# dell-research-harvard/effocr

Measured on AMD Instinct MI355X. Metric: glyph-crops/sec end-to-end (encode+kNN), 224x224 bs=1024, higher is better.
Workload: dtype bf16; 1 GPU; BASELINE configs[1]: vit_small_patch16_224 encoder (bf16 MFMA operands, fp32 accumulate/residual/LN/softmax), 1024x3x224x224 fp32 crops per GPU resident in HBM, 10000-row fp32 IndexFlatIP, k=10; seeded random-init weights; crops_per_gpu=1024, global_batch=1024, index_rows=10000, k=10, parallelism=1024 crops per GPU, weights+index replicated

## Files before the change

### effocr_amd/_lib.py

```python
import ctypes
import os
import subprocess
import threading

_HERE = os.path.dirname(os.path.abspath(__file__))
_CSRC = os.path.join(_HERE, "csrc")
SO_PATH = os.environ.get("EFFOCR_HIP_LIB") or os.path.join(_HERE, "libeffocr_hip.so")
SO_PATH_AB = os.path.join(_HERE, "libeffocr_hip_ab.so")

ABI_VERSION = 9
PREC = {"bf16": 0, "fp16": 1, "fp32": 2}
EPI = {"bias": 0, "bias_gelu": 1, "bias_resid": 2}

_lock = threading.Lock()
_lib = None
_loaded = {}


class EffOCRHipError(RuntimeError):
    pass


def build(force=False, verbose=False, ab=True):
    so = os.path.join(_HERE, "libeffocr_hip.so")
# ... 84 lines not shown
        "effocr_letterbox": (i32, [vp, i32, i32, i64, i32, i32, i32, i32, i32, i32, i32, f32p, vp]),
        "effocr_nms_workspace_bytes": (sz, [i32, i32]),
        "effocr_nms_batch_workspace_bytes": (sz, [i32, i32, i32]),
        "effocr_nms": (i32, [f32p, i32, i32, c.c_float, c.c_float, i32, i32, c.c_float, i32, f32p, vp, vp, sz, vp]),
        "effocr_nms_batch": (i32, [f32p, i32, i32, i32, c.c_float, c.c_float, i32, i32, c.c_float, i32, f32p, vp, vp, sz, vp]),
        "effocr_parse_char_boxes": (i32, [f32p, vp, i32, i32, i32, i32, i32, i32, f32p, vp, vp, vp, vp]),
        "effocr_op_linear": (i32, [i32, i32, vp, vp, f32p, f32p, vp, i32, i32, i32, vp]),
        "effocr_op_layernorm": (i32, [i32, f32p, i64, i32, f32p, f32p, c.c_float, vp, vp]),
        "effocr_op_attention": (i32, [i32, vp, vp, i32, i32, i32, vp]),
        "effocr_op_linear_blocked": (i32, [i32, i32, vp, vp, f32p, f32p, vp, i32, i32, i32, i32, vp]),
        "effocr_op_mlp_blocked": (i32, [i32, f32p, f32p, f32p, c.c_float, vp, f32p, vp, f32p, f32p, i32, i32, i32, i32, vp, sz, vp]),
        "effocr_op_mlp_ln_blocked": (i32, [i32, f32p, f32p, f32p, c.c_float, vp, f32p, vp, f32p, f32p, f32p, f32p, vp, i32, i32, i32, i32, vp, sz, vp]),
        "effocr_op_proj_mlp_blocked": (i32, [i32, f32p, vp, vp, f32p, f32p, f32p, c.c_float, vp, f32p, vp, f32p, f32p, i32, i32, i32, i32, vp, sz, vp]),
        "effocr_op_qkv_attn_blocked": (i32, [i32, vp, vp, f32p, vp, i32, i32, i32, i32, vp]),
        "effocr_op_layernorm_blocked": (i32, [i32, f32p, i64, i32, f32p, f32p, c.c_float, vp, vp]),
    }
    for name, (res, args) in sig.items():
        if os.environ.get("EFFOCR_HIP_LIB") and not hasattr(lib, name):
            def _absent(*a, _n=name, **k):
                raise EffOCRHipError(f"{_n} is not exported by the library EFFOCR_HIP_LIB points at")
            setattr(lib, name, _absent)
            continue
        fn = getattr(lib, name)
        fn.restype = res
        fn.argtypes = args
    return sig


EXPORTS = None

# ... 380 lines not shown
```

### effocr_amd/csrc/api.hip

```cpp
#include "../../include/effocr_hip.h"
#include "enc_core.hpp"


#include <math.h>
#include <algorithm>
#include <string.h>
#include <map>
#include <memory>
#include <string>
#include <vector>

namespace effocr {

namespace {

struct Param { std::string name; std::vector<int64_t> shape; int64_t numel; std::vector<float> data; bool set; };

struct VitCfg { int D, depth, heads, mlp; };
struct VitLayerOff { size_t ln1w, ln1b, qkvb, projb, ln2w, ln2b, fc1b, fc2b, qkvw, projw, fc1w, fc2w;
                     size_t qkvw_b, projw_b, fc1w_b, fc2w_b, projw_pp, fc2w_pp, projb_p, fc2b_p, qkvw_bv, qkvb_v;
                     size_t qkvw_bf, qkv_s, qkv_c, fc1w_bf, fc1_s, fc1_c; };
struct ConvSpec { std::string w, bn; int cin, cout, k, stride, pad; size_t w_off, b_off; };
struct CnxBlockOff { size_t dww, dwb, lnw, lnb, w1, b1, w2, b2, gamma; };
struct CnxStageOff { int C, Cp, depth; size_t dslnw, dslnb, dsw, dsb; std::vector<CnxBlockOff> blocks; };

}
}

using namespace effocr;

struct effocr_encoder {
  std::string arch;
  bool is_vit = false;
  int img = 224, prec = PREC_BF16, D = 0;
  std::vector<Param> params;
  std::map<std::string, int> index;
  VitCfg vit{};
  int T = 0, P = 0;
  size_t off_clspos0 = 0, off_pos = 0, off_patchb = 0, off_normw = 0, off_normb = 0, off_patchw = 0, off_patchw_b = 0;
  std::vector<VitLayerOff> layers;
  std::vector<ConvSpec> convs;
  bool is_cnx = false;
  std::vector<CnxStageOff> cnx;
  size_t cnx_stemw = 0, cnx_stemb = 0, cnx_stemlnw = 0, cnx_stemlnb = 0, cnx_headw = 0, cnx_headb = 0;
  bool is_mnv = false;
  MnvNet mnv{};
  size_t wbytes = 0;
  const char* wdev = nullptr;
  int debug = 0;
  int cls_only_last = 1;
  int mlp_stagger_min_rounds = 2;
  int mlp_tail_first = 96;
  int mlp_stagger = 2500;
  int use_projf = 1;
  int use_qkvattn = 1;
  int qa_min_batch = 1;
  int qa_hsplit = 0;
  int use_patchf = 1;
  int use_mlp = 1;
  int use_gemm3 = 1;
  int use_lnfold = 1;
  int tail_split = 1;
  int split6 = 1;
  int pair_parts = 1;
  int mlp_pair = 0;
  int use_blocked = 1;
  int use_gemm2 = 1;
  int panel_rows = 128;
  int use_panel = 1;
  int chunk = 0;
  int call_size_invariant = 0;
  int prof_mode = 0;
// ... 60 lines not shown
    L.ln2w = a.take((size_t)D * 4); L.ln2b = a.take((size_t)D * 4);
    L.fc1b = a.take((size_t)mlp * 4); L.fc2b = a.take((size_t)D * 4);
  }
  e->off_normw = a.take((size_t)D * 4);
  e->off_normb = a.take((size_t)D * 4);
  e->off_patchw = a.take((size_t)D * 768 * es);
  for (int i = 0; i < depth; ++i) {
    VitLayerOff& L = e->layers[i];
    L.qkvw = a.take((size_t)3 * D * D * es);
    L.projw = a.take((size_t)D * D * es);
    L.fc1w = a.take((size_t)mlp * D * es);
    L.fc2w = a.take((size_t)D * mlp * es);
  }
  if (e->prec != PREC_FP32) {
    e->off_patchw_b = a.take((size_t)D * 768 * es);
    for (int i = 0; i < depth; ++i) {
      VitLayerOff& L = e->layers[i];
      L.fc2w_b = a.take((size_t)D * mlp * es);
      L.fc2w_pp = a.take((size_t)D * mlp * es);
      L.projw_pp = a.take((size_t)D * D * es);
      L.projb_p = a.take((size_t)D * 4);
      L.fc2b_p = a.take((size_t)D * 4);
      L.qkvw_bv = a.take((size_t)3 * D * D * es);
      L.qkvb_v = a.take((size_t)3 * D * 4);
      {
        L.qkvw_b = a.take((size_t)3 * D * D * es);
        L.projw_b = a.take((size_t)D * D * es);
        L.fc1w_b = a.take((size_t)mlp * D * es);
        L.qkvw_bf = a.take((size_t)3 * D * D * es); L.qkv_s = a.take((size_t)3 * D * 4); L.qkv_c = a.take((size_t)3 * D * 4);
        L.fc1w_bf = a.take((size_t)mlp * D * es); L.fc1_s = a.take((size_t)mlp * 4); L.fc1_c = a.take((size_t)mlp * 4);
// ... 391 lines not shown
  }
  const int cls = prof_class(e, name);
  const size_t slot = e->prof_used++;
  const bool clk = e->prof_mode == 1 && slot < effocr_encoder::PROF_CLK_SLOTS &&
                   (e->prof_clk || hipMalloc(&e->prof_clk, effocr_encoder::PROF_CLK_SLOTS * 8192 * sizeof(unsigned long long)) == hipSuccess && hipMemset(e->prof_clk, 0, effocr_encoder::PROF_CLK_SLOTS * 8192 * sizeof(unsigned long long)) == hipSuccess);
  if (clk) (void)clock_sample(e->prof_clk + slot * 8192, s);
  (void)hipEventRecord(e->prof_pool[slot].first, s);
  const int rc = launch();
  (void)hipEventRecord(e->prof_pool[slot].second, s);
  if (clk) (void)clock_sample(e->prof_clk + slot * 8192 + 4096, s);
  e->prof_rec.push_back({cls, (int)slot});
  e->prof_work[cls] += work;
  return rc;
}

struct VitWs { size_t status, x, xn, qkv, att, h, stats, total, rows, hbytes; };
VitWs vit_ws(const effocr_encoder* e, int B) {
  const size_t M = align_up((size_t)B * e->T, 128), D = e->vit.D, es = prec_esize(e->prec);
  Alloc a; VitWs w;
  w.rows = M;
  w.status = a.take(256);
  w.x = a.take(M * D * 4);
  w.xn = a.take(M * D * es);
  w.qkv = a.take(M * 3 * D * es);
  w.att = a.take(M * D * es);
  size_t hb = M * e->vit.mlp * es, pb = (size_t)B * e->P * 768 * es;
  w.hbytes = hb > pb ? hb : pb;
  {
    const size_t cus = (size_t)device_cus(), np = M / 128, tail = np % cus;
    const size_t split = (tail && tail * 6 <= cus) ? 6 : (tail && tail * 4 <= cus) ? 4 : (tail && tail * 2 <= cus) ? 2 : 0;
// ... 14 lines not shown
  void* xn = ws + w.xn; void* qkv = ws + w.qkv; void* att = ws + w.att; void* hb = ws + w.h;
  auto F = [&](size_t off) { return reinterpret_cast<const float*>(wb + off); };
  int rc;
  const double Md = (double)M, Dd = (double)D, Hd = (double)e->vit.mlp;
  const bool panel = e->use_panel && panel_gemm_supported(prec, 3 * D, D) && panel_gemm_supported(prec, e->vit.mlp, D);
  const bool g2 = e->use_gemm2 && gemm2_supported(prec, D, e->vit.mlp);
  const bool g2p = e->use_gemm2 && gemm2_supported(prec, D, 768);
  const bool g3all = !panel && e->use_gemm3 && gemm3_supported(prec, 3 * D, D) && gemm3_supported(prec, D, D) &&
                     gemm3_supported(prec, e->vit.mlp, D) && gemm3_supported(prec, D, e->vit.mlp);
  const int blk = (e->use_blocked && g2p && ((panel && g2) || g3all)) ? 1 : 0;
  const bool mlpf = blk && panel && e->use_mlp && mlp_fused_supported(prec, D, e->vit.mlp);
  const bool projf = mlpf && e->use_projf;
  const bool qaf = blk && panel && mlpf && qkv_attn_supported(prec, D, T) && (e->use_qkvattn == 2 || (e->use_qkvattn == 1 && (e->call_size_invariant || B >= e->qa_min_batch)));
  const bool g3 = blk && e->use_gemm3 && gemm3_supported(prec, D, e->vit.mlp);
  const bool patchf = blk && e->use_patchf && patch_embed_fused_supported(prec, D);
  if (!patchf && (rc = timed(e, "im2col_patch16", 0.0, s, [&] { return im2col_patch16(prec, x, x16, B, e->img, e->img, hb, s); }))) return rc;
  int* status = reinterpret_cast<int*>(ws + w.status);
  if (!patchf && (rc = set_cls_rows(F(e->off_clspos0), xs, B, T, D, blk, nullptr, s))) return rc;
  GemmArgs g{};
  if (patchf) {
    PatchArgs pa{};
    pa.x = x; pa.x16 = x16; pa.B = B; pa.H = e->img; pa.W = e->img; pa.Wb = wb + e->off_patchw_b; pa.bias = F(e->off_patchb); pa.pos = F(e->off_pos);
    pa.out = xs; pa.D = D; pa.P = Pn; pa.cls = F(e->off_clspos0);
    if ((rc = timed(e, "patch_embed_fused", 2.0 * B * Pn * Dd * 768.0, s, [&] { return patch_embed_fused(prec, pa, s); }))) return rc;
  } else {
  g.X = hb; g.ldx = 768; g.W = wb + e->off_patchw; g.ldw = 768; g.bias = F(e->off_patchb);
  g.out = xs; g.ldo = D; g.pos = F(e->off_pos); g.M = B * Pn; g.N = D; g.K = 768; g.P = Pn; g.blk_out = blk;
  if ((rc = timed(e, "gemm_patch_embed", 2.0 * B * Pn * Dd * 768.0, s, [&] { return g2p ? gemm2_nt(prec, EPI_PATCH, g, s) : gemm_nt(prec, EPI_PATCH, g, s); }))) return rc;
  }
  const float* cls_x = nullptr;
  bool xn_ready = false;
  for (int i = 0; i < e->vit.depth; ++i) {
    const VitLayerOff& L = e->layers[i];
    if (panel) {
      {
      PanelArgs p{};
      if (qaf) {
        if (!xn_ready && (rc = timed(e, "layernorm", 0.0, s, [&] { return layernorm_rows_blocked(prec, xs, M, D, F(L.ln1w), F(L.ln1b), 1e-6f, xn, s); }))) return rc;
        xn_ready = false;
        QkvAttnArgs q{};
        q.xn = xn; q.Wb = wb + L.qkvw_bv; q.bias = F(L.qkvb_v); q.out = att;
        q.B = B; q.T = T; q.D = D; q.rows_alloc = (int64_t)w.rows; q.hsplit = e->qa_hsplit;
        q.cls_only = (i + 1 == e->vit.depth && e->cls_only_last && projf) ? 1 : 0;
        const bool cls_k = q.cls_only && D == 384 && T > 192;
        const double qa_work = cls_k ? 2.0 * Md * 2.0 * Dd * Dd + 2.0 * (32.0 * B) * Dd * Dd + 4.0 * B * e->vit.heads * 32.0 * T * 64.0
                                     : 2.0 * Md * 3.0 * Dd * Dd + 4.0 * B * e->vit.heads * (double)T * T * 64.0;
// ... 402 lines not shown
}

size_t effocr_encoder_weights_bytes(const effocr_encoder_t* enc) { return enc ? enc->wbytes : 0; }

int effocr_encoder_upload(effocr_encoder_t* enc, void* weights_dev, size_t bytes) {
  if (!enc || !weights_dev) return fail(EFFOCR_EINVAL, "upload: NULL argument");
  if (bytes < enc->wbytes) return fail(EFFOCR_EWORKSPACE, "upload: weight buffer too small");
  for (const Param& p : enc->params)
    if (!p.set) return fail(EFFOCR_ESTATE, "upload: parameter '" + p.name + "' was never set");
  std::vector<char> blob(enc->wbytes, 0);
  if (enc->is_vit) pack_vit(enc, blob); else if (enc->is_cnx) pack_convnext(enc, blob); else if (enc->is_mnv) pack_mobilenetv3(enc, blob);
  else pack_resnet(enc, blob);
  const hipError_t er = hipMemcpy(weights_dev, blob.data(), enc->wbytes, hipMemcpyHostToDevice);
  if (er != hipSuccess) return fail(EFFOCR_EHIP, std::string("upload: hipMemcpy: ") + hipGetErrorString(er));
  enc->wdev = static_cast<const char*>(weights_dev);
  return EFFOCR_OK;
}

size_t effocr_encoder_workspace_bytes(const effocr_encoder_t* enc, int batch) {
  if (!enc || batch <= 0) return 0;
  if (enc->is_cnx) return convnext_ws(enc, cnx_chunk(enc, batch)).total;
  if (enc->is_mnv) return mnv3_ws(enc, mnv3_chunk(enc, batch)).total;
  if (!enc->is_vit) return resnet_ws(enc, batch).total;
  return vit_ws(enc, (enc->chunk > 0 && enc->chunk < batch) ? enc->chunk : batch).total;
}

int effocr_encoder_set_option(effocr_encoder_t* enc, const char* name, int value) {
  if (!enc || !name) return fail(EFFOCR_EINVAL, "set_option: NULL argument");
  const std::string n = name;
  if (n == "use_panel") { enc->use_panel = value; return EFFOCR_OK; }
  if (n == "debug") { enc->debug = value; return EFFOCR_OK; }
  if (n == "use_gemm2") { enc->use_gemm2 = value; return EFFOCR_OK; }
  if (n == "use_blocked") { enc->use_blocked = value; return EFFOCR_OK; }
  if (n == "tail_split") { enc->tail_split = value; return EFFOCR_OK; }
  if (n == "split6") { enc->split6 = value; return EFFOCR_OK; }
  if (n == "mlp_pair") { enc->mlp_pair = value; return EFFOCR_OK; }
  if (n == "pair_parts") { enc->pair_parts = value; return EFFOCR_OK; }
  if (n == "use_gemm3") { enc->use_gemm3 = value; return EFFOCR_OK; }
  if (n == "use_lnfold") { enc->use_lnfold = value; return EFFOCR_OK; }
  if (n == "use_mlp") { enc->use_mlp = value; return EFFOCR_OK; }
  if (n == "use_qkvattn") { enc->use_qkvattn = value; return EFFOCR_OK; }
  if (n == "qa_min_batch") { enc->qa_min_batch = value; return EFFOCR_OK; }
  if (n == "qa_hsplit") { enc->qa_hsplit = value; return EFFOCR_OK; }
  if (n == "use_patchf") { enc->use_patchf = value; return EFFOCR_OK; }
  if (n == "use_projf") { enc->use_projf = value; return EFFOCR_OK; }
  if (n == "cls_only_last") { enc->cls_only_last = value; return EFFOCR_OK; }
  if (n == "mlp_stagger_min_rounds") { enc->mlp_stagger_min_rounds = value < 1 ? 1 : value; return EFFOCR_OK; }
  if (n == "mlp_tail_first") { enc->mlp_tail_first = value < 0 ? 0 : value & ~7; return EFFOCR_OK; }
  if (n == "mlp_stagger") { enc->mlp_stagger = value < 0 ? 0 : value; return EFFOCR_OK; }
  if (n == "panel_rows") { if (value != 64 && value != 128) return fail(EFFOCR_EINVAL, "set_option: panel_rows must be 64 or 128"); enc->panel_rows = value; return EFFOCR_OK; }
  if (n == "call_size_invariant") {
    if (value != 0 && value != 1) return fail(EFFOCR_EINVAL, "set_option: call_size_invariant must be 0 or 1");
    enc->call_size_invariant = value; return EFFOCR_OK;
  }
  if (n == "chunk") { if (value < 0) return fail(EFFOCR_EINVAL, "set_option: chunk < 0"); enc->chunk = value; return EFFOCR_OK; }
  return fail(EFFOCR_EINVAL, "set_option: unknown option '" + n + "'");
}

int effocr_encoder_set_chunk(effocr_encoder_t* enc, int crops_per_chunk) {
// ... 331 lines not shown
  if (batch > 0 && (!xn_blk_dev || !wqkv_blk_dev || !bias_dev || !out_blk_dev))
    return fail(EFFOCR_EINVAL, "op_qkv_attn_blocked: NULL device pointer");
  if (batch < 0 || tokens < 1) return fail(EFFOCR_EINVAL, "op_qkv_attn_blocked: bad batch / tokens");
  QkvAttnArgs q{};
  q.xn = xn_blk_dev; q.Wb = wqkv_blk_dev; q.bias = bias_dev; q.out = out_blk_dev;
  q.B = batch; q.T = tokens; q.D = d; q.rows_alloc = rows_alloc;
  return qkv_attn_fused(precision, q, S(stream));
}

int effocr_op_layernorm_blocked(int out_precision, const float* x_blk_dev, int64_t rows, int d, const float* gamma_dev,
                                const float* beta_dev, float eps, void* out_blk_dev, void* stream) {
  if (rows > 0 && (!x_blk_dev || !gamma_dev || !beta_dev || !out_blk_dev)) return fail(EFFOCR_EINVAL, "op_layernorm_blocked: NULL device pointer");
  return layernorm_rows_blocked(out_precision, x_blk_dev, rows, d, gamma_dev, beta_dev, eps, out_blk_dev, S(stream));
}

int effocr_op_layernorm(int out_precision, const float* x_dev, int64_t rows, int d, const float* gamma_dev,
                        const float* beta_dev, float eps, void* out_dev, void* stream) {
  return layernorm_rows(out_precision, x_dev, rows, d, gamma_dev, beta_dev, eps, out_dev, S(stream));
}

int effocr_op_attention(int precision, const void* qkv_dev, void* out_dev, int batch, int tokens, int heads, void* stream) {
  return attention(precision, qkv_dev, out_dev, batch, tokens, heads, 0, S(stream));
}

}
```

### effocr_amd/csrc/kernels.hpp

```cpp
#pragma once
#include "common.hpp"

namespace effocr {

enum { PREC_BF16 = 0, PREC_FP16 = 1, PREC_FP32 = 2 };
enum { EPI_BIAS = 0, EPI_BIAS_GELU = 1, EPI_BIAS_RESID = 2, EPI_PATCH = 3,
       EPI_BIAS_SCALE_RESID = 4,
       EPI_BIAS_F32 = 5 };

static inline int prec_esize(int prec) { return prec == PREC_FP32 ? 4 : 2; }

struct GemmArgs {
  const void* X; int64_t ldx;
  const void* W; int64_t ldw;
  const float* bias;
  void* out; int64_t ldo;
  const float* resid; int64_t ldr;
  const float* pos;
  int M, N, K;
  int P;
  int blk_x;
  int blk_out;
  const void* Wblk;
  int rows_alloc;
// ... 43 lines not shown
  int cls_only;
  int img0;
  int hsplit;
};
bool qkv_attn_supported(int prec, int D, int T);
int qkv_attn_fused(int prec, const QkvAttnArgs& a, hipStream_t s);

struct PatchArgs {
  const void* x; int B, H, W;
  int x16;
  const void* Wb;
  const float* bias; const float* pos;
  const float* cls;
  float* out;
  int D, P;
};
bool patch_embed_fused_supported(int prec, int D);
int patch_embed_fused(int prec, const PatchArgs& a, hipStream_t s);

enum { PRO_COPY = 0, PRO_LN = 1 };
struct PanelArgs {
  const void* A; int64_t lda;
  const float* gamma; const float* beta; float eps;
  const void* W;
  const float* bias;
  void* out; int64_t ldo;
  const float* resid; int64_t ldr;
  int M, N, K;
  unsigned long long* dbg;
  int debug;
  int blk_a;
  int blk_out;
// ... 109 lines not shown
```

### effocr_amd/csrc/ln.hpp

```cpp
#pragma once
#include "common.hpp"

namespace effocr {

template <int G> __device__ __forceinline__ float group_sum(float v) {
#pragma unroll
  for (int o = G / 2; o >= 1; o >>= 1) v += __shfl_xor(v, o, 64);
  return v;
}

template <int G, int V>
__device__ __forceinline__ void ln_apply(const f32x4 (&v)[V], int sub, const float* __restrict__ gamma,
                                         const float* __restrict__ beta, float eps, f32x4 (&y)[V]) {
  constexpr int D = 4 * G * V;
  float s = 0.f;
#pragma unroll
  for (int i = 0; i < V; ++i) s += (v[i][0] + v[i][1]) + (v[i][2] + v[i][3]);
  const float mean = group_sum<G>(s) * (1.0f / D);
  float ss = 0.f;
#pragma unroll
  for (int i = 0; i < V; ++i) {
#pragma unroll
    for (int e = 0; e < 4; ++e) { const float d = v[i][e] - mean; ss += d * d; }
  }
  const float var = group_sum<G>(ss) * (1.0f / D);
  const float rstd = 1.0f / sqrtf(var + eps);
#pragma unroll
  for (int i = 0; i < V; ++i) {
    const f32x4 gm = *reinterpret_cast<const f32x4*>(gamma + (sub + G * i) * 4);
    const f32x4 bt = *reinterpret_cast<const f32x4*>(beta + (sub + G * i) * 4);
#pragma unroll
    for (int e = 0; e < 4; ++e) y[i][e] = (v[i][e] - mean) * rstd * gm[e] + bt[e];
  }
}

template <int G, int V>
__device__ __forceinline__ void ln_row(const float* __restrict__ xr, int sub, const float* __restrict__ gamma,
                                       const float* __restrict__ beta, float eps, f32x4 (&y)[V]) {
  f32x4 v[V];
#pragma unroll
  for (int i = 0; i < V; ++i) v[i] = *reinterpret_cast<const f32x4*>(xr + (sub + G * i) * 4);
  ln_apply<G, V>(v, sub, gamma, beta, eps, y);
}

}
```

### effocr_amd/csrc/patch.hip

```cpp
#include "common.hpp"
#include "kernels.hpp"
#include <type_traits>

constexpr int PE_SLABS = 2;
constexpr int PE_SLABS16 = 4;
#ifndef PATCH_NT
#define PATCH_NT 1
#endif
namespace effocr {
#ifdef EFFOCR_CONVOPS
thread_local int convops_patch_dw = 0, convops_patch_grid = 0;
#define PATCH_REC(dw, grid) (convops_patch_dw = (dw), convops_patch_grid = (int)(grid))
#else
#define PATCH_REC(dw, grid) ((void)0)
#endif
namespace {

template <int I, int N, typename F> __device__ __forceinline__ void pfor(F&& f) {
  if constexpr (I < N) {
    f(std::integral_constant<int, I>{});
    pfor<I + 1, N>(f);
  }
}

// ... 4 lines not shown
template <typename E, typename X, int D>
__global__ __launch_bounds__(256, 1) void patch_embed_kernel(PatchArgs a) {
  typedef typename Op16<E>::V8 V8;
  constexpr bool X16 = sizeof(X) == 2;
  constexpr int NSL = X16 ? PE_SLABS16 : PE_SLABS;
  constexpr int KC = PE_K / 8;
  constexpr int OT = D / 32, OG = OT / 4;
  constexpr int KS = PE_K / 64;
  constexpr int NS = KS * OG;
  constexpr int R = PE_RING;
  static_assert(D % 128 == 0 && D <= 384, "patch_embed: a workgroup's output slice must be 128, 256 or 384 wide");
  static_assert(NS >= R - 1, "patch_embed: the panel's stream must be at least as long as the prefetch distance");
  __shared__ __attribute__((aligned(16))) char smem[R * PE_STAGE];
  const int tid = threadIdx.x, lane = tid & 63, r31 = lane & 31, half = lane >> 5;
  const int w = wave_id();
  const int64_t total = (int64_t)a.B * a.P;
  const int nsl = a.D / D;
  const int panel = (int)blockIdx.x / nsl, n0 = ((int)blockIdx.x - panel * nsl) * D;
  const int64_t m = (int64_t)panel * 128 + w * 32 + r31;
  const int64_t mc = m < total ? m : total - 1;
  const int img = (int)(mc / a.P), p = (int)(mc - (int64_t)img * a.P);
  const int PW = a.W / 16, ty = p / PW, tx = p - ty * PW;
  const X* xp = static_cast<const X*>(a.x) + ((int64_t)img * 3 * a.H + ty * 16) * a.W + tx * 16 + 8 * half;
  const int64_t plane = (int64_t)a.H * a.W;

  struct Slab { u32x4 v[X16 ? 4 : 8]; };
  auto load_slab = [&](Slab& sl, int ks) __attribute__((always_inline)) {
#pragma unroll
    for (int c4 = 0; c4 < 4; ++c4) {
      const int kk = ks * 4 + c4;
// ... 69 lines not shown
  WF wf;
  asm volatile("s_waitcnt vmcnt(%0)" ::"n"((R - 2) * 4) : "memory");
  __builtin_amdgcn_s_barrier();
  asm volatile("" ::: "memory");
#pragma unroll
  for (int i = 0; i < 4; ++i) wf.w[i] = *reinterpret_cast<const V8*>(smem + wo + (i * 8) * 512);

  pfor<0, NS>([&](auto S_) {
    constexpr int S = decltype(S_)::value;
    constexpr int ks = S / OG, g = S % OG;
    constexpr bool more = S + R - 1 < NS, next = S + 1 < NS;
    const char* st = smem + (S & (R - 1)) * PE_STAGE;
    const char* stn = smem + ((S + 1) & (R - 1)) * PE_STAGE;
    if constexpr (g == 0) {
      to_frags(sl[ks % NSL], xf);
      if constexpr (ks + NSL < KS) load_slab(sl[ks % NSL], ks + NSL);
    }
    pfor<0, 4>([&](auto C4) {
      constexpr int c4 = decltype(C4)::value;
      if constexpr (c4 == 2) {
        if constexpr (S + R - 2 < NS) asm volatile("s_waitcnt vmcnt(%0)" ::"n"((R - 3) * 4) : "memory");
        else asm volatile("s_waitcnt vmcnt(0)" ::: "memory");
        __builtin_amdgcn_s_barrier();
        asm volatile("" ::: "memory");
      }
      pfor<0, 4>([&](auto I) {
        constexpr int i = decltype(I)::value;
        acc[4 * g + i] = Op16<E>::mfma(wf.w[i], xf[c4], acc[4 * g + i]);
        __builtin_amdgcn_sched_barrier(0);
        if constexpr (c4 < 3) wf.w[i] = *reinterpret_cast<const V8*>(st + wo + (i * 8 + 2 * (c4 + 1)) * 512);
        else if constexpr (next) wf.w[i] = *reinterpret_cast<const V8*>(stn + wo + (i * 8) * 512);
        if constexpr (more && c4 == 2 && i == 0) issue_stage_asm(S + R - 1);
      });
    });
  });

  if (m < total) {
    const int64_t orow = (int64_t)img * (a.P + 1) + 1 + p;
    const float* posr = a.pos + (int64_t)(1 + p) * a.D + n0;
    const float* biasr = a.bias + n0;
    char* ob = reinterpret_cast<char*>(a.out) + ((orow >> 5) * (a.D >> 2) + (n0 >> 2)) * 512 + (orow & 31) * 16;
    pfor<0, OT>([&](auto T_) {
      constexpr int t = decltype(T_)::value;
#pragma unroll
      for (int q = 0; q < 4; ++q) {
        const int f0 = 32 * t + 8 * q + 4 * half;
        const f32x4 bv = *reinterpret_cast<const f32x4*>(biasr + f0);
        const f32x4 pv = *reinterpret_cast<const f32x4*>(posr + f0);
        const f32x4 o = {acc[t][4 * q] + bv[0] + pv[0], acc[t][4 * q + 1] + bv[1] + pv[1], acc[t][4 * q + 2] + bv[2] + pv[2],
                         acc[t][4 * q + 3] + bv[3] + pv[3]};
        if (PATCH_NT & 2) __builtin_nontemporal_store(o, reinterpret_cast<f32x4*>(ob + (f0 >> 2) * 512)); else *reinterpret_cast<f32x4*>(ob + (f0 >> 2) * 512) = o;
      }
    });
    if (a.cls != nullptr && p == 0) {
      const int64_t crow = orow - 1;
      char* cb = reinterpret_cast<char*>(a.out) + ((crow >> 5) * (a.D >> 2) + (n0 >> 2)) * 512 + (crow & 31) * 16;
      for (int c = half; c < D / 4; c += 2)
        *reinterpret_cast<f32x4*>(cb + c * 512) = *reinterpret_cast<const f32x4*>(a.cls + n0 + 4 * c);
    }
  }
}

template <typename E, typename X>
int launch_patch(const PatchArgs& a, hipStream_t s) {
  const int64_t total = (int64_t)a.B * a.P;
  const int64_t panels = (total + 127) / 128;
  if (a.D == 384 && panels * 3 <= device_cus()) {
    PATCH_REC(128, panels * 3);
    hipLaunchKernelGGL((patch_embed_kernel<E, X, 128>), dim3((unsigned)(panels * 3)), dim3(256), 0, s, a);
    return check_launch("patch_embed_fused");
  }
  const int nsl = a.D > 384 ? a.D / 384 : 1;
  const dim3 grid((unsigned)(panels * nsl)), blk(256);
  switch (a.D) {
    case 128: PATCH_REC(128, grid.x); hipLaunchKernelGGL((patch_embed_kernel<E, X, 128>), grid, blk, 0, s, a); break;
    case 256: PATCH_REC(256, grid.x); hipLaunchKernelGGL((patch_embed_kernel<E, X, 256>), grid, blk, 0, s, a); break;
    case 384: case 768: PATCH_REC(384, grid.x); hipLaunchKernelGGL((patch_embed_kernel<E, X, 384>), grid, blk, 0, s, a); break;
    default: return fail(EFFOCR_EUNSUPPORTED, "patch_embed_fused: embed dim must be 128, 256, 384 or 768");
  }
  return check_launch("patch_embed_fused");
}

}

bool patch_embed_fused_supported(int prec, int D) { return (prec == PREC_BF16 || prec == PREC_FP16) && (D == 128 || D == 256 || D == 384 || D == 768); }

int patch_embed_fused(int prec, const PatchArgs& a, hipStream_t s) {
  if (a.B <= 0) return EFFOCR_OK;
  if (!patch_embed_fused_supported(prec, a.D)) return fail(EFFOCR_EUNSUPPORTED, "patch_embed_fused: needs bf16/fp16 and an embed dim of 128, 256, 384 or 768");
  if (a.H % 16 || a.W % 16 || a.P != (a.H / 16) * (a.W / 16)) return fail(EFFOCR_EINVAL, "patch_embed_fused: image size must be a multiple of 16");
  if (a.x16) return prec == PREC_BF16 ? launch_patch<__bf16, __bf16>(a, s) : launch_patch<_Float16, _Float16>(a, s);
  return prec == PREC_BF16 ? launch_patch<__bf16, float>(a, s) : launch_patch<_Float16, float>(a, s);
}

}
```

### effocr_amd/csrc/vit_ops.hip

```cpp
#include "common.hpp"
#include "kernels.hpp"
#include "ln.hpp"
#include <math.h>


#ifndef ATT_NT
#define ATT_NT 0
#endif
#ifndef LN_NT
#define LN_NT 1
#endif
namespace effocr {
namespace {

template <int G, int V, typename TO>
__global__ __launch_bounds__(256) void layernorm_kernel(const float* __restrict__ x, int64_t rows,
                                                        const float* __restrict__ gamma,
                                                        const float* __restrict__ beta, float eps,
                                                        TO* __restrict__ out) {
  constexpr int D = 4 * G * V;
  constexpr int RPW = 64 / G;
  const int lane = threadIdx.x & 63, sub = lane % G;
  const int64_t row = ((int64_t)blockIdx.x * 4 + (threadIdx.x >> 6)) * RPW + lane / G;
  const int64_t rc = row < rows ? row : rows - 1;
// ... 59 lines not shown
        for (int e = 0; e < 4; ++e) acc[e] += pv[e];
      }
      const f32x4 bv = *reinterpret_cast<const f32x4*>(rd.b2 + c * 4);
      f32x4 xo = {0.f, 0.f, 0.f, 0.f};
      if (rd.add_x) xo = *reinterpret_cast<const f32x4*>(xb + (size_t)c * 512);
#pragma unroll
      for (int e = 0; e < 4; ++e) v[i][e] = acc[e] + bv[e] + (rd.add_x ? xo[e] : 0.f);
      if (live) *reinterpret_cast<f32x4*>(reinterpret_cast<char*>(rd.xw) + rb * (D / 4) * 512 + tl * 16 + (size_t)c * 512) = v[i];
    }
  } else {
#pragma unroll
    for (int i = 0; i < NQ; ++i) v[i] = (LN_NT & 1) ? __builtin_nontemporal_load(reinterpret_cast<const f32x4*>(xb + (size_t)(c0 + 2 * i) * 512)) : *reinterpret_cast<const f32x4*>(xb + (size_t)(c0 + 2 * i) * 512);
  }
  float s = 0.f;
#pragma unroll
  for (int i = 0; i < NQ; ++i) s += (v[i][0] + v[i][1]) + (v[i][2] + v[i][3]);
  s += __shfl_xor(s, 32, 64);
  if (part == 0) red[0][wv][tl] = s;
  __syncthreads();
  const float mean = ((red[0][0][tl] + red[0][1][tl]) + (red[0][2][tl] + red[0][3][tl])) * (1.0f / D);
  float ss = 0.f;
#pragma unroll
  for (int i = 0; i < NQ; ++i)
#pragma unroll
    for (int e = 0; e < 4; ++e) { const float d = v[i][e] - mean; ss += d * d; }
  ss += __shfl_xor(ss, 32, 64);
  if (part == 0) red[1][wv][tl] = ss;
  __syncthreads();
  const float var = ((red[1][0][tl] + red[1][1][tl]) + (red[1][2][tl] + red[1][3][tl])) * (1.0f / D);
  const float rstd = 1.0f / sqrtf(var + eps);
  if (rb * 32 + tl >= rows) return;
  char* ob = reinterpret_cast<char*>(out) + rb * (D / 8) * 512 + tl * 16 + part * 8;
#pragma unroll
  for (int i = 0; i < NQ; ++i) {
    const int c = c0 + 2 * i;
    const f32x4 gm = REDUCE ? gmv[REDUCE ? i : 0] : *reinterpret_cast<const f32x4*>(gamma + c * 4);
    const f32x4 bt = REDUCE ? btv[REDUCE ? i : 0] : *reinterpret_cast<const f32x4*>(beta + c * 4);
    const u32x2 o = pack4<TO>((v[i][0] - mean) * rstd * gm[0] + bt[0], (v[i][1] - mean) * rstd * gm[1] + bt[1],
                              (v[i][2] - mean) * rstd * gm[2] + bt[2], (v[i][3] - mean) * rstd * gm[3] + bt[3]);
    if (LN_NT & 2) __builtin_nontemporal_store(o, reinterpret_cast<u32x2*>(ob + (size_t)(c >> 1) * 512));
    else *reinterpret_cast<u32x2*>(ob + (size_t)(c >> 1) * 512) = o;
  }
}

template <int G, int V>
__global__ __launch_bounds__(256) void cls_norm_kernel(const float* __restrict__ x, int B, int T,
                                                       const float* __restrict__ gamma,
                                                       const float* __restrict__ beta, float eps, int l2norm,
                                                       int blocked, float* __restrict__ emb, int* __restrict__ status) {
  constexpr int D = 4 * G * V;
  constexpr int RPW = 64 / G;
  const int lane = threadIdx.x & 63, sub = lane % G;
  const int img = (blockIdx.x * 4 + (threadIdx.x >> 6)) * RPW + lane / G;
  const int ic = img < B ? img : B - 1;
// ... 469 lines not shown
```

### include/effocr_hip.h

```cpp
#ifndef EFFOCR_HIP_H
#define EFFOCR_HIP_H

#include <stddef.h>
#include <stdint.h>

#ifdef __cplusplus
extern "C" {
#endif

#define EFFOCR_ABI_VERSION 9

enum effocr_status {
  EFFOCR_OK = 0,
  EFFOCR_EINVAL = -1,
  EFFOCR_EUNSUPPORTED = -2,
  EFFOCR_EWORKSPACE = -3,
  EFFOCR_EHIP = -4,
  EFFOCR_ESTATE = -5,
  EFFOCR_EOVERFLOW = -6
};

enum effocr_precision {
  EFFOCR_PREC_BF16 = 0,
  EFFOCR_PREC_FP16 = 1,
// ... 114 lines not shown
                          int m, int d, int h, int rows_alloc, void* scratch_dev, size_t scratch_bytes, void* stream);
int effocr_op_mlp_ln_blocked(int precision, float* x_blk_dev, const float* gamma_dev, const float* beta_dev, float eps,
                             const void* w1_blk_dev, const float* b1_dev, const void* w2_perm_dev, const float* b2_perm_dev, const float* b2_dev,
                             const float* gamma_next_dev, const float* beta_next_dev, void* xn_blk_dev,
                             int m, int d, int h, int rows_alloc, void* scratch_dev, size_t scratch_bytes, void* stream);
int effocr_op_proj_mlp_blocked(int precision, float* x_blk_dev, const void* a_blk_dev, const void* wp_perm_dev, const float* bp_perm_dev,
                               const float* gamma_dev, const float* beta_dev, float eps, const void* w1_blk_dev, const float* b1_dev,
                               const void* w2_perm_dev, const float* b2_perm_dev, const float* b2_dev, int m, int d, int h, int rows_alloc,
                               void* scratch_dev, size_t scratch_bytes, void* stream);

int effocr_op_qkv_attn_blocked(int precision, const void* xn_blk_dev, const void* wqkv_blk_dev, const float* bias_dev,
                               void* out_blk_dev, int batch, int tokens, int d, int rows_alloc, void* stream);
int effocr_op_layernorm_blocked(int out_precision, const float* x_blk_dev, int64_t rows, int d, const float* gamma_dev,
                                const float* beta_dev, float eps, void* out_blk_dev, void* stream);

#ifdef __cplusplus
}
#endif
#endif
```

Baseline: 96420 glyph-crops/s.

## Fuse layer-0 norm1 LayerNorm into patch-embed epilogue with precomputed class-token row

The patch-embed kernel now computes the first block's LayerNorm over each full 384-wide row in its epilogue and writes the normalised bf16 activations directly. The class-token row's normalised value is precomputed once at weight upload and copied in. This drops the separate layer-0 LN kernel and the round trip of re-reading the fp32 residual stream. It adds register pressure and extra stores to the patch kernel. It also adds an optional, off-by-default workgroup launch stagger and diagnostic macros, and refactors the LN arithmetic into shared helpers with explicit FMA ordering so the fused and standalone paths match.

New measurement: 97110 glyph-crops/s (median of 6 runs). No clear change (+0.7%).

```diff
diff --git a/effocr_amd/_lib.py b/effocr_amd/_lib.py
--- a/effocr_amd/_lib.py
+++ b/effocr_amd/_lib.py
@@ -122,6 +122,7 @@
         "effocr_op_proj_mlp_blocked": (i32, [i32, f32p, vp, vp, f32p, f32p, f32p, c.c_float, vp, f32p, vp, f32p, f32p, i32, i32, i32, i32, vp, sz, vp]),
         "effocr_op_qkv_attn_blocked": (i32, [i32, vp, vp, f32p, vp, i32, i32, i32, i32, vp]),
         "effocr_op_layernorm_blocked": (i32, [i32, f32p, i64, i32, f32p, f32p, c.c_float, vp, vp]),
+        "effocr_op_patch_embed_blocked": (i32, [i32, vp, i32, i32, i32, i32, vp, f32p, f32p, f32p, f32p, i32, i32, vp, f32p, f32p, c.c_float, vp, i32, vp]),
     }
     for name, (res, args) in sig.items():
         if os.environ.get("EFFOCR_HIP_LIB") and not hasattr(lib, name):
diff --git a/effocr_amd/csrc/api.hip b/effocr_amd/csrc/api.hip
--- a/effocr_amd/csrc/api.hip
+++ b/effocr_amd/csrc/api.hip
@@ -38,6 +38,7 @@
   VitCfg vit{};
   int T = 0, P = 0;
   size_t off_clspos0 = 0, off_pos = 0, off_patchb = 0, off_normw = 0, off_normb = 0, off_patchw = 0, off_patchw_b = 0;
+  size_t off_clsxn = 0;
   std::vector<VitLayerOff> layers;
   std::vector<ConvSpec> convs;
   bool is_cnx = false;
@@ -56,6 +57,8 @@
   int use_qkvattn = 1;
   int qa_min_batch = 1;
   int qa_hsplit = 0;
+  int patch_norm1 = 1;
+  int patch_stagger = 0;
   int use_patchf = 1;
   int use_mlp = 1;
   int use_gemm3 = 1;
@@ -146,6 +149,7 @@
   }
   if (e->prec != PREC_FP32) {
     e->off_patchw_b = a.take((size_t)D * 768 * es);
+    if (D == 384) e->off_clsxn = a.take((size_t)D * es);
     for (int i = 0; i < depth; ++i) {
       VitLayerOff& L = e->layers[i];
       L.fc2w_b = a.take((size_t)D * mlp * es);
@@ -567,6 +571,25 @@
   return rc;
 }
 
+int upload_cls_norm1(effocr_encoder* e, char* wdev) {
+  const int D = e->vit.D;
+  const size_t xbytes = (size_t)(D / 4) * 512, obytes = (size_t)(D / 8) * 512;
+  char* tmp = nullptr;
+  if (hipMalloc(&tmp, xbytes + obytes) != hipSuccess) return fail(EFFOCR_EHIP, "upload: hipMalloc (class-token norm1)");
+  int rc = EFFOCR_OK;
+  if (hipMemset(tmp, 0, xbytes + obytes) != hipSuccess ||
+      hipMemcpy2D(tmp, 512, wdev + e->off_clspos0, 16, 16, D / 4, hipMemcpyDeviceToDevice) != hipSuccess)
+    rc = fail(EFFOCR_EHIP, "upload: class-token row");
+  if (!rc) rc = layernorm_rows_blocked(e->prec, reinterpret_cast<const float*>(tmp), 1, D, reinterpret_cast<const float*>(wdev + e->layers[0].ln1w),
+                                       reinterpret_cast<const float*>(wdev + e->layers[0].ln1b), 1e-6f, tmp + xbytes, nullptr);
+  if (!rc && (hipStreamSynchronize(nullptr) != hipSuccess ||
+              hipMemcpy2D(wdev + e->off_clsxn, 16, tmp + xbytes, 512, 16, D / 8, hipMemcpyDeviceToDevice) != hipSuccess ||
+              hipDeviceSynchronize() != hipSuccess))
+    rc = fail(EFFOCR_EHIP, "upload: class-token norm1");
+  (void)hipFree(tmp);
+  return rc;
+}
+
 struct VitWs { size_t status, x, xn, qkv, att, h, stats, total, rows, hbytes; };
 VitWs vit_ws(const effocr_encoder* e, int B) {
   const size_t M = align_up((size_t)B * e->T, 128), D = e->vit.D, es = prec_esize(e->prec);
@@ -611,6 +634,7 @@
   const bool qaf = blk && panel && mlpf && qkv_attn_supported(prec, D, T) && (e->use_qkvattn == 2 || (e->use_qkvattn == 1 && (e->call_size_invariant || B >= e->qa_min_batch)));
   const bool g3 = blk && e->use_gemm3 && gemm3_supported(prec, D, e->vit.mlp);
   const bool patchf = blk && e->use_patchf && patch_embed_fused_supported(prec, D);
+  const bool pn1 = patchf && qaf && e->patch_norm1 && e->off_clsxn && e->vit.depth > 0 && patch_embed_norm1_supported(prec, D, (int64_t)B * Pn);
   if (!patchf && (rc = timed(e, "im2col_patch16", 0.0, s, [&] { return im2col_patch16(prec, x, x16, B, e->img, e->img, hb, s); }))) return rc;
   int* status = reinterpret_cast<int*>(ws + w.status);
   if (!patchf && (rc = set_cls_rows(F(e->off_clspos0), xs, B, T, D, blk, nullptr, s))) return rc;
@@ -618,7 +642,10 @@
   if (patchf) {
     PatchArgs pa{};
     pa.x = x; pa.x16 = x16; pa.B = B; pa.H = e->img; pa.W = e->img; pa.Wb = wb + e->off_patchw_b; pa.bias = F(e->off_patchb); pa.pos = F(e->off_pos);
-    pa.out = xs; pa.D = D; pa.P = Pn; pa.cls = F(e->off_clspos0);
+    pa.out = xs; pa.D = D; pa.P = Pn; pa.cls = F(e->off_clspos0); pa.stagger = e->patch_stagger;
+    if (pn1) {
+      pa.xn_out = xn; pa.gamma = F(e->layers[0].ln1w); pa.beta = F(e->layers[0].ln1b); pa.eps = 1e-6f; pa.cls_xn = wb + e->off_clsxn;
+    }
     if ((rc = timed(e, "patch_embed_fused", 2.0 * B * Pn * Dd * 768.0, s, [&] { return patch_embed_fused(prec, pa, s); }))) return rc;
   } else {
   g.X = hb; g.ldx = 768; g.W = wb + e->off_patchw; g.ldw = 768; g.bias = F(e->off_patchb);
@@ -626,7 +653,7 @@
   if ((rc = timed(e, "gemm_patch_embed", 2.0 * B * Pn * Dd * 768.0, s, [&] { return g2p ? gemm2_nt(prec, EPI_PATCH, g, s) : gemm_nt(prec, EPI_PATCH, g, s); }))) return rc;
   }
   const float* cls_x = nullptr;
-  bool xn_ready = false;
+  bool xn_ready = pn1;
   for (int i = 0; i < e->vit.depth; ++i) {
     const VitLayerOff& L = e->layers[i];
     if (panel) {
@@ -1059,6 +1086,7 @@
   const hipError_t er = hipMemcpy(weights_dev, blob.data(), enc->wbytes, hipMemcpyHostToDevice);
   if (er != hipSuccess) return fail(EFFOCR_EHIP, std::string("upload: hipMemcpy: ") + hipGetErrorString(er));
   enc->wdev = static_cast<const char*>(weights_dev);
+  if (enc->is_vit && enc->off_clsxn) return upload_cls_norm1(enc, static_cast<char*>(weights_dev));
   return EFFOCR_OK;
 }
 
@@ -1088,6 +1116,8 @@
   if (n == "qa_min_batch") { enc->qa_min_batch = value; return EFFOCR_OK; }
   if (n == "qa_hsplit") { enc->qa_hsplit = value; return EFFOCR_OK; }
   if (n == "use_patchf") { enc->use_patchf = value; return EFFOCR_OK; }
+  if (n == "patch_norm1") { if (value != 0 && value != 1) return fail(EFFOCR_EINVAL, "set_option: patch_norm1 must be 0 or 1"); enc->patch_norm1 = value; return EFFOCR_OK; }
+  if (n == "patch_stagger") { enc->patch_stagger = value < 0 ? 0 : value; return EFFOCR_OK; }
   if (n == "use_projf") { enc->use_projf = value; return EFFOCR_OK; }
   if (n == "cls_only_last") { enc->cls_only_last = value; return EFFOCR_OK; }
   if (n == "mlp_stagger_min_rounds") { enc->mlp_stagger_min_rounds = value < 1 ? 1 : value; return EFFOCR_OK; }
@@ -1449,6 +1479,18 @@
   return layernorm_rows_blocked(out_precision, x_blk_dev, rows, d, gamma_dev, beta_dev, eps, out_blk_dev, S(stream));
 }
 
+int effocr_op_patch_embed_blocked(int precision, const void* x_dev, int x16, int batch, int h, int w, const void* w_blk_dev, const float* bias_dev,
+                                  const float* pos_dev, const float* cls_dev, float* out_blk_dev, int d, int patches, void* xn_blk_dev,
+                                  const float* gamma_dev, const float* beta_dev, float eps, const void* cls_xn_dev, int stagger, void* stream) {
+  if (!x_dev || !w_blk_dev || !bias_dev || !pos_dev || !out_blk_dev) return fail(EFFOCR_EINVAL, "op_patch_embed_blocked: NULL device pointer");
+  if (batch < 0 || h < 16 || w < 16 || d < 1 || patches < 1) return fail(EFFOCR_EINVAL, "op_patch_embed_blocked: bad shape");
+  if ((int64_t)batch * (patches + 1) >= (int64_t)1 << 31 || (int64_t)batch * 3 * h * w >= (int64_t)1 << 40) return fail(EFFOCR_EUNSUPPORTED, "op_patch_embed_blocked: batch too large");
+  PatchArgs a{};
+  a.x = x_dev; a.x16 = x16 ? 1 : 0; a.B = batch; a.H = h; a.W = w; a.Wb = w_blk_dev; a.bias = bias_dev; a.pos = pos_dev; a.cls = cls_dev; a.out = out_blk_dev;
+  a.D = d; a.P = patches; a.xn_out = xn_blk_dev; a.gamma = gamma_dev; a.beta = beta_dev; a.eps = eps; a.cls_xn = cls_xn_dev; a.stagger = stagger < 0 ? 0 : stagger;
+  return patch_embed_fused(precision, a, S(stream));
+}
+
 int effocr_op_layernorm(int out_precision, const float* x_dev, int64_t rows, int d, const float* gamma_dev,
                         const float* beta_dev, float eps, void* out_dev, void* stream) {
   return layernorm_rows(out_precision, x_dev, rows, d, gamma_dev, beta_dev, eps, out_dev, S(stream));
diff --git a/effocr_amd/csrc/kernels.hpp b/effocr_amd/csrc/kernels.hpp
--- a/effocr_amd/csrc/kernels.hpp
+++ b/effocr_amd/csrc/kernels.hpp
@@ -81,8 +81,12 @@
   const float* cls;
   float* out;
   int D, P;
+  void* xn_out; const float* gamma; const float* beta; float eps; const void* cls_xn;
+  int stagger;
+  int stagger_wgs;
 };
 bool patch_embed_fused_supported(int prec, int D);
+bool patch_embed_norm1_supported(int prec, int D, int64_t patches);
 int patch_embed_fused(int prec, const PatchArgs& a, hipStream_t s);
 
 enum { PRO_COPY = 0, PRO_LN = 1 };
diff --git a/effocr_amd/csrc/ln.hpp b/effocr_amd/csrc/ln.hpp
--- a/effocr_amd/csrc/ln.hpp
+++ b/effocr_amd/csrc/ln.hpp
@@ -34,6 +34,30 @@
   }
 }
 
+__device__ __forceinline__ float lnb_add4(float s, const f32x4& v) { return s + ((v[0] + v[1]) + (v[2] + v[3])); }
+__device__ __forceinline__ float lnb_sum4(float q0, float q1, float q2, float q3) { return (q0 + q1) + (q2 + q3); }
+template <int D> __device__ __forceinline__ float lnb_mean(float S) {
+#pragma clang fp contract(off)
+  return S * (1.0f / D);
+}
+template <int D, bool FIRST> __device__ __forceinline__ float lnb_addsq4(float ss, const f32x4& v, float S) {
+#pragma clang fp contract(off)
+  const float d0 = __builtin_fmaf(S, -(1.0f / D), v[0]), d1 = __builtin_fmaf(S, -(1.0f / D), v[1]);
+  const float d2 = __builtin_fmaf(S, -(1.0f / D), v[2]), d3 = __builtin_fmaf(S, -(1.0f / D), v[3]);
+  ss = FIRST ? __builtin_fmaf(d0, d0, d1 * d1) : __builtin_fmaf(d1, d1, __builtin_fmaf(d0, d0, ss));
+  return __builtin_fmaf(d3, d3, __builtin_fmaf(d2, d2, ss));
+}
+template <int D> __device__ __forceinline__ float lnb_rstd(float SS, float eps) {
+#pragma clang fp contract(off)
+  return 1.0f / sqrtf(__builtin_fmaf(SS, 1.0f / D, eps));
+}
+template <typename TO>
+__device__ __forceinline__ u32x2 lnb_out4(const f32x4& v, float mean, float rstd, const f32x4& gm, const f32x4& bt) {
+#pragma clang fp contract(off)
+  return pack4<TO>(__builtin_fmaf((v[0] - mean) * rstd, gm[0], bt[0]), __builtin_fmaf((v[1] - mean) * rstd, gm[1], bt[1]),
+                   __builtin_fmaf((v[2] - mean) * rstd, gm[2], bt[2]), __builtin_fmaf((v[3] - mean) * rstd, gm[3], bt[3]));
+}
+
 template <int G, int V>
 __device__ __forceinline__ void ln_row(const float* __restrict__ xr, int sub, const float* __restrict__ gamma,
                                        const float* __restrict__ beta, float eps, f32x4 (&y)[V]) {
diff --git a/effocr_amd/csrc/patch.hip b/effocr_amd/csrc/patch.hip
--- a/effocr_amd/csrc/patch.hip
+++ b/effocr_amd/csrc/patch.hip
@@ -1,11 +1,15 @@
 #include "common.hpp"
 #include "kernels.hpp"
+#include "ln.hpp"
 #include <type_traits>
 
 constexpr int PE_SLABS = 2;
 constexpr int PE_SLABS16 = 4;
 #ifndef PATCH_NT
 #define PATCH_NT 1
+#endif
+#ifndef PATCH_DIAG
+#define PATCH_DIAG 0
 #endif
 namespace effocr {
 #ifdef EFFOCR_CONVOPS
@@ -42,6 +46,10 @@
   __shared__ __attribute__((aligned(16))) char smem[R * PE_STAGE];
   const int tid = threadIdx.x, lane = tid & 63, r31 = lane & 31, half = lane >> 5;
   const int w = wave_id();
+  if (a.stagger > 0 && (int)blockIdx.x < a.stagger_wgs) {
+    const unsigned long long until = __builtin_amdgcn_s_memtime() + (unsigned long long)((((int)blockIdx.x >> 3) & 31) * a.stagger);
+    while (__builtin_amdgcn_s_memtime() < until) __builtin_amdgcn_s_sleep(8);
+  }
   const int64_t total = (int64_t)a.B * a.P;
   const int nsl = a.D / D;
   const int panel = (int)blockIdx.x / nsl, n0 = ((int)blockIdx.x - panel * nsl) * D;
@@ -141,7 +149,7 @@
     const char* stn = smem + ((S + 1) & (R - 1)) * PE_STAGE;
     if constexpr (g == 0) {
       to_frags(sl[ks % NSL], xf);
-      if constexpr (ks + NSL < KS) load_slab(sl[ks % NSL], ks + NSL);
+      if constexpr (ks + NSL < KS && !(PATCH_DIAG & 2)) load_slab(sl[ks % NSL], ks + NSL);
     }
     pfor<0, 4>([&](auto C4) {
       constexpr int c4 = decltype(C4)::value;
@@ -153,7 +161,8 @@
       }
       pfor<0, 4>([&](auto I) {
         constexpr int i = decltype(I)::value;
-        acc[4 * g + i] = Op16<E>::mfma(wf.w[i], xf[c4], acc[4 * g + i]);
+        if constexpr (!(PATCH_DIAG & 4)) acc[4 * g + i] = Op16<E>::mfma(wf.w[i], xf[c4], acc[4 * g + i]);
+        else asm volatile("" ::"v"(wf.w[i]), "v"(xf[c4]));
         __builtin_amdgcn_sched_barrier(0);
         if constexpr (c4 < 3) wf.w[i] = *reinterpret_cast<const V8*>(st + wo + (i * 8 + 2 * (c4 + 1)) * 512);
         else if constexpr (next) wf.w[i] = *reinterpret_cast<const V8*>(stn + wo + (i * 8) * 512);
@@ -162,28 +171,119 @@
     });
   });
 
+  const bool xn = D == 384 && a.xn_out != nullptr && a.D == 384;
+  __syncthreads();
+  {
+    f32x4* sv = reinterpret_cast<f32x4*>(smem);
+    if (tid < D / 4) {
+      sv[tid] = *reinterpret_cast<const f32x4*>(a.bias + n0 + 4 * tid);
+      if constexpr (D == 384) {
+        if (xn) {
+          sv[96 + tid] = *reinterpret_cast<const f32x4*>(a.gamma + 4 * tid);
+          sv[192 + tid] = *reinterpret_cast<const f32x4*>(a.beta + 4 * tid);
+        }
+      }
+    }
+  }
+  __syncthreads();
   if (m < total) {
+    const f32x4* sv = reinterpret_cast<const f32x4*>(smem);
+    const float* posr = a.pos + (int64_t)(1 + p) * a.D + n0;
+    constexpr int GT = OT % 3 == 0 ? 3 : 2;
+    pfor<0, OT / GT>([&](auto G_) {
+      constexpr int t0 = decltype(G_)::value * GT;
+      f32x4 pvs[GT * 4];
+#pragma unroll
+      for (int i = 0; i < GT * 4; ++i) pvs[i] = *reinterpret_cast<const f32x4*>(posr + 32 * (t0 + i / 4) + 8 * (i % 4) + 4 * half);
+      pfor<0, GT>([&](auto T_) {
+        constexpr int t = t0 + decltype(T_)::value;
+#pragma unroll
+        for (int q = 0; q < 4; ++q) {
+          const f32x4 bv = sv[8 * t + 2 * q + half], pv = pvs[(t - t0) * 4 + q];
+          const f32x4 o = {acc[t][4 * q] + bv[0] + pv[0], acc[t][4 * q + 1] + bv[1] + pv[1], acc[t][4 * q + 2] + bv[2] + pv[2],
+                           acc[t][4 * q + 3] + bv[3] + pv[3]};
+#pragma unroll
+          for (int e = 0; e < 4; ++e) acc[t][4 * q + e] = o[e];
+        }
+      });
+    });
     const int64_t orow = (int64_t)img * (a.P + 1) + 1 + p;
-    const float* posr = a.pos + (int64_t)(1 + p) * a.D + n0;
-    const float* biasr = a.bias + n0;
-    char* ob = reinterpret_cast<char*>(a.out) + ((orow >> 5) * (a.D >> 2) + (n0 >> 2)) * 512 + (orow & 31) * 16;
-    pfor<0, OT>([&](auto T_) {
-      constexpr int t = decltype(T_)::value;
-#pragma unroll
-      for (int q = 0; q < 4; ++q) {
-        const int f0 = 32 * t + 8 * q + 4 * half;
-        const f32x4 bv = *reinterpret_cast<const f32x4*>(biasr + f0);
-        const f32x4 pv = *reinterpret_cast<const f32x4*>(posr + f0);
-        const f32x4 o = {acc[t][4 * q] + bv[0] + pv[0], acc[t][4 * q + 1] + bv[1] + pv[1], acc[t][4 * q + 2] + bv[2] + pv[2],
-                         acc[t][4 * q + 3] + bv[3] + pv[3]};
-        if (PATCH_NT & 2) __builtin_nontemporal_store(o, reinterpret_cast<f32x4*>(ob + (f0 >> 2) * 512)); else *reinterpret_cast<f32x4*>(ob + (f0 >> 2) * 512) = o;
-      }
-    });
+    if constexpr (!(PATCH_DIAG & 1)) {
+      char* ob = reinterpret_cast<char*>(a.out) + ((orow >> 5) * (a.D >> 2) + (n0 >> 2)) * 512 + (orow & 31) * 16;
+      pfor<0, OT>([&](auto T_) {
+        constexpr int t = decltype(T_)::value;
+#pragma unroll
+        for (int q = 0; q < 4; ++q) {
+          const f32x4 o = {acc[t][4 * q], acc[t][4 * q + 1], acc[t][4 * q + 2], acc[t][4 * q + 3]};
+          f32x4* dst = reinterpret_cast<f32x4*>(ob + (8 * t + 2 * q + half) * 512);
+          if (PATCH_NT & 2) __builtin_nontemporal_store(o, dst); else *dst = o;
+        }
+      });
+    }
+    if constexpr (D == 384) {
+      if (xn) {
+        float qs[4];
+        pfor<0, 4>([&](auto WV) {
+          constexpr int wv = decltype(WV)::value;
+          float sq = 0.f;
+          pfor<3 * wv, 3 * wv + 3>([&](auto T_) {
+            constexpr int t = decltype(T_)::value;
+#pragma unroll
+            for (int q = 0; q < 4; ++q) sq = lnb_add4(sq, f32x4{acc[t][4 * q], acc[t][4 * q + 1], acc[t][4 * q + 2], acc[t][4 * q + 3]});
+          });
+          sq += __shfl_xor(sq, 32, 64);
+          qs[wv] = sq;
+        });
+        const float S = lnb_sum4(qs[0], qs[1], qs[2], qs[3]);
+        pfor<0, 4>([&](auto WV) {
+          constexpr int wv = decltype(WV)::value;
+          float sq = 0.f;
+          pfor<3 * wv, 3 * wv + 3>([&](auto T_) {
+            constexpr int t = decltype(T_)::value;
+            pfor<0, 4>([&](auto Q_) {
+              constexpr int q = decltype(Q_)::value;
+              sq = lnb_addsq4<384, t == 3 * wv && q == 0>(sq, f32x4{acc[t][4 * q], acc[t][4 * q + 1], acc[t][4 * q + 2], acc[t][4 * q + 3]}, S);
+            });
+          });
+          sq += __shfl_xor(sq, 32, 64);
+          qs[wv] = sq;
+        });
+        const float mean = lnb_mean<384>(S);
+        const float rstd = lnb_rstd<384>(lnb_sum4(qs[0], qs[1], qs[2], qs[3]), a.eps);
+        char* xb = reinterpret_cast<char*>(a.xn_out) + (orow >> 5) * (384 / 8) * 512 + (orow & 31) * 16 + half * 8;
+        pfor<0, OT>([&](auto T_) {
+          constexpr int t = decltype(T_)::value;
+#pragma unroll
+          for (int q = 0; q < 4; ++q) {
+            const int c = 8 * t + 2 * q + half;
+            *reinterpret_cast<u32x2*>(xb + (4 * t + q) * 512) =
+                lnb_out4<E>(f32x4{acc[t][4 * q], acc[t][4 * q + 1], acc[t][4 * q + 2], acc[t][4 * q + 3]}, mean, rstd, sv[96 + c], sv[192 + c]);
+          }
+        });
+      }
+    }
     if (a.cls != nullptr && p == 0) {
       const int64_t crow = orow - 1;
       char* cb = reinterpret_cast<char*>(a.out) + ((crow >> 5) * (a.D >> 2) + (n0 >> 2)) * 512 + (crow & 31) * 16;
-      for (int c = half; c < D / 4; c += 2)
-        *reinterpret_cast<f32x4*>(cb + c * 512) = *reinterpret_cast<const f32x4*>(a.cls + n0 + 4 * c);
+      constexpr int CB = 16;
+#pragma unroll
+      for (int c0 = 0; c0 < D / 8; c0 += CB) {
+        f32x4 cv[CB];
+#pragma unroll
+        for (int i = 0; i < CB; ++i) cv[i] = *reinterpret_cast<const f32x4*>(a.cls + n0 + 4 * (half + 2 * (c0 + i)));
+#pragma unroll
+        for (int i = 0; i < CB; ++i) *reinterpret_cast<f32x4*>(cb + (half + 2 * (c0 + i)) * 512) = cv[i];
+      }
+      if constexpr (D == 384) {
+        if (xn) {
+          char* xcb = reinterpret_cast<char*>(a.xn_out) + (crow >> 5) * (384 / 8) * 512 + (crow & 31) * 16;
+          u32x4 cx[24];
+#pragma unroll
+          for (int i = 0; i < 24; ++i) cx[i] = *reinterpret_cast<const u32x4*>(static_cast<const char*>(a.cls_xn) + 16 * (half + 2 * i));
+#pragma unroll
+          for (int i = 0; i < 24; ++i) *reinterpret_cast<u32x4*>(xcb + (half + 2 * i) * 512) = cx[i];
+        }
+      }
     }
   }
 }
@@ -193,21 +293,35 @@
   const int64_t total = (int64_t)a.B * a.P;
   const int64_t panels = (total + 127) / 128;
   if (a.D == 384 && panels * 3 <= device_cus()) {
+    if (a.xn_out != nullptr) return fail(EFFOCR_EUNSUPPORTED, "patch_embed_fused: the norm1 output needs whole-width panels (this call runs 128-wide slices)");
     PATCH_REC(128, panels * 3);
-    hipLaunchKernelGGL((patch_embed_kernel<E, X, 128>), dim3((unsigned)(panels * 3)), dim3(256), 0, s, a);
+    PatchArgs b = a;
+    b.stagger_wgs = 0;
+    hipLaunchKernelGGL((patch_embed_kernel<E, X, 128>), dim3((unsigned)(panels * 3)), dim3(256), 0, s, b);
     return check_launch("patch_embed_fused");
+  }
+  if (a.xn_out != nullptr) {
+    if (a.D != 384) return fail(EFFOCR_EUNSUPPORTED, "patch_embed_fused: the norm1 output needs whole-width panels at an embed dim of 384");
+    if (!a.gamma || !a.beta || (a.cls && !a.cls_xn)) return fail(EFFOCR_EINVAL, "patch_embed_fused: the norm1 output needs gamma, beta and (with cls) the normalised cls row");
   }
   const int nsl = a.D > 384 ? a.D / 384 : 1;
   const dim3 grid((unsigned)(panels * nsl)), blk(256);
+  PatchArgs b = a;
+  if (b.stagger > (1 << 20)) b.stagger = 1 << 20;
+  b.stagger_wgs = (b.stagger > 0 && (int64_t)grid.x >= 2 * (int64_t)device_cus()) ? device_cus() : 0;
   switch (a.D) {
-    case 128: PATCH_REC(128, grid.x); hipLaunchKernelGGL((patch_embed_kernel<E, X, 128>), grid, blk, 0, s, a); break;
-    case 256: PATCH_REC(256, grid.x); hipLaunchKernelGGL((patch_embed_kernel<E, X, 256>), grid, blk, 0, s, a); break;
-    case 384: case 768: PATCH_REC(384, grid.x); hipLaunchKernelGGL((patch_embed_kernel<E, X, 384>), grid, blk, 0, s, a); break;
+    case 128: PATCH_REC(128, grid.x); hipLaunchKernelGGL((patch_embed_kernel<E, X, 128>), grid, blk, 0, s, b); break;
+    case 256: PATCH_REC(256, grid.x); hipLaunchKernelGGL((patch_embed_kernel<E, X, 256>), grid, blk, 0, s, b); break;
+    case 384: case 768: PATCH_REC(384, grid.x); hipLaunchKernelGGL((patch_embed_kernel<E, X, 384>), grid, blk, 0, s, b); break;
     default: return fail(EFFOCR_EUNSUPPORTED, "patch_embed_fused: embed dim must be 128, 256, 384 or 768");
   }
   return check_launch("patch_embed_fused");
 }
 
+}
+
+bool patch_embed_norm1_supported(int prec, int D, int64_t patches) {
+  return (prec == PREC_BF16 || prec == PREC_FP16) && D == 384 && patches > 0 && ((patches + 127) / 128) * 3 > device_cus();
 }
 
 bool patch_embed_fused_supported(int prec, int D) { return (prec == PREC_BF16 || prec == PREC_FP16) && (D == 128 || D == 256 || D == 384 || D == 768); }
diff --git a/effocr_amd/csrc/vit_ops.hip b/effocr_amd/csrc/vit_ops.hip
--- a/effocr_amd/csrc/vit_ops.hip
+++ b/effocr_amd/csrc/vit_ops.hip
@@ -97,21 +97,19 @@
   }
   float s = 0.f;
 #pragma unroll
-  for (int i = 0; i < NQ; ++i) s += (v[i][0] + v[i][1]) + (v[i][2] + v[i][3]);
+  for (int i = 0; i < NQ; ++i) s = lnb_add4(s, v[i]);
   s += __shfl_xor(s, 32, 64);
   if (part == 0) red[0][wv][tl] = s;
   __syncthreads();
-  const float mean = ((red[0][0][tl] + red[0][1][tl]) + (red[0][2][tl] + red[0][3][tl])) * (1.0f / D);
-  float ss = 0.f;
-#pragma unroll
-  for (int i = 0; i < NQ; ++i)
-#pragma unroll
-    for (int e = 0; e < 4; ++e) { const float d = v[i][e] - mean; ss += d * d; }
+  const float S = lnb_sum4(red[0][0][tl], red[0][1][tl], red[0][2][tl], red[0][3][tl]);
+  float ss = lnb_addsq4<D, true>(0.f, v[0], S);
+#pragma unroll
+  for (int i = 1; i < NQ; ++i) ss = lnb_addsq4<D, false>(ss, v[i], S);
   ss += __shfl_xor(ss, 32, 64);
   if (part == 0) red[1][wv][tl] = ss;
   __syncthreads();
-  const float var = ((red[1][0][tl] + red[1][1][tl]) + (red[1][2][tl] + red[1][3][tl])) * (1.0f / D);
-  const float rstd = 1.0f / sqrtf(var + eps);
+  const float mean = lnb_mean<D>(S);
+  const float rstd = lnb_rstd<D>(lnb_sum4(red[1][0][tl], red[1][1][tl], red[1][2][tl], red[1][3][tl]), eps);
   if (rb * 32 + tl >= rows) return;
   char* ob = reinterpret_cast<char*>(out) + rb * (D / 8) * 512 + tl * 16 + part * 8;
 #pragma unroll
@@ -119,8 +117,7 @@
     const int c = c0 + 2 * i;
     const f32x4 gm = REDUCE ? gmv[REDUCE ? i : 0] : *reinterpret_cast<const f32x4*>(gamma + c * 4);
     const f32x4 bt = REDUCE ? btv[REDUCE ? i : 0] : *reinterpret_cast<const f32x4*>(beta + c * 4);
-    const u32x2 o = pack4<TO>((v[i][0] - mean) * rstd * gm[0] + bt[0], (v[i][1] - mean) * rstd * gm[1] + bt[1],
-                              (v[i][2] - mean) * rstd * gm[2] + bt[2], (v[i][3] - mean) * rstd * gm[3] + bt[3]);
+    const u32x2 o = lnb_out4<TO>(v[i], mean, rstd, gm, bt);
     if (LN_NT & 2) __builtin_nontemporal_store(o, reinterpret_cast<u32x2*>(ob + (size_t)(c >> 1) * 512));
     else *reinterpret_cast<u32x2*>(ob + (size_t)(c >> 1) * 512) = o;
   }
diff --git a/include/effocr_hip.h b/include/effocr_hip.h
--- a/include/effocr_hip.h
+++ b/include/effocr_hip.h
@@ -152,6 +152,10 @@
 int effocr_op_layernorm_blocked(int out_precision, const float* x_blk_dev, int64_t rows, int d, const float* gamma_dev,
                                 const float* beta_dev, float eps, void* out_blk_dev, void* stream);
 
+int effocr_op_patch_embed_blocked(int precision, const void* x_dev, int x16, int batch, int h, int w, const void* w_blk_dev, const float* bias_dev,
+                                  const float* pos_dev, const float* cls_dev, float* out_blk_dev, int d, int patches, void* xn_blk_dev,
+                                  const float* gamma_dev, const float* beta_dev, float eps, const void* cls_xn_dev, int stagger, void* stream);
+
 #ifdef __cplusplus
 }
 #endif
```
